# xiph/daala

Measured on AMD Instinct MI355X. Metric: 1080p all-intra transform blocks/s (filter+DCT+PVQ), higher is better.
Workload: dtype int32 (lifting DCT/filters) + f64 (PVQ search)

## Files before the change

### daala_amd/csrc/pvq_refbands.hip

```cpp
#include "../../include/daala_hip.h"
#include <math.h>
#include <stdio.h>
#include <stdlib.h>
#include <string.h>
#include "od_ctx.cuh"
#include "od_pvq_math.cuh"
#include "od_occupancy.cuh"
#include "od_krange.cuh"
#include "od_band_stage.cuh"
#include "gen/od_scan_tables.h"
#define OD_RSQ_TABLE_N 512
#define OD_RSQ_HUGE
#include "pvq_search.cuh"
#include "pvq_row.cuh"
#include "pvq_regs.cuh"

namespace {

constexpr int kMaxJobs = 8;
constexpr int kMaxItems = kMaxJobs*ODHIP_MAX_BANDS;
constexpr int kSlots = ODHIP_PVQ_REF_SLOTS;
constexpr int kUncCap = 1 << 16;
constexpr double kDefaultMargin = 1e-9;

struct RJob {
  const od_coeff *coef;
  const od_coeff *ref;
  const int16_t *qm;
  const int16_t *qm_inv;
  odhip_pvq_refband *rec;
  void *items;
  int16_t *y;
  int16_t *r16;
  int16_t *x16;
  int16_t *xr;
  const double *rate;
  int32_t *choice;
  od_coeff *dq;
  unsigned short *keys;
  unsigned *ids;
  unsigned *krange;
  long nblocks;
  int nplanes;
  int w;
  int h;
  int bs;
  int nb_bands;
  int len;
  int bw;
  int bh;
  int is_keyframe;
  int pli;
  int q[ODHIP_MAX_BANDS];
  int beta[ODHIP_MAX_BANDS];
  int off[ODHIP_MAX_BANDS + 1];
  long split_blk;
  int q2[ODHIP_MAX_BANDS];
  const int *qp;
  unsigned plane_blocks;
  const int16_t *ly;
  const int32_t *lchoice;
  const int16_t *lqmi;
  long lnblocks;
  long lsplit;
  int llen;
  int lnb;
};

__device__ __forceinline__ int job_q(const RJob &jb, int band, long blk) {
  const int q = blk >= jb.split_blk ? jb.q2[band] : jb.q[band];
  return q ? q : jb.qp[(unsigned)blk/jb.plane_blocks*ODHIP_MAX_BANDS + band];
}

__device__ __forceinline__ void lref_piece(const RJob &jb, int band, long blk, int c0, int (&rv)[8]) {
  const long lblk = blk >= jb.lsplit ? blk - jb.lsplit : blk;
  const int4 ch = reinterpret_cast<const int4 *>(jb.lchoice)[lblk*jb.lnb + band];
  uint4 y4 = make_uint4(0, 0, 0, 0);
  if (ch.y != 0) y4 = *reinterpret_cast<const uint4 *>(jb.ly + ((long)ch.x*jb.lnblocks + lblk)*jb.llen + c0);
  const uint4 q4 = *reinterpret_cast<const uint4 *>(jb.lqmi + c0);
  const unsigned yw[4] = {y4.x, y4.y, y4.z, y4.w};
  const unsigned qw[4] = {q4.x, q4.y, q4.z, q4.w};
#pragma unroll
  for (int e = 0; e < 8; e++) {
    const int yv = (int16_t)(yw[e >> 1] >> (16*(e & 1)));
    const int qmi = (int16_t)(qw[e >> 1] >> (16*(e & 1)));
    rv[e] = odq_shr_round(odq_mult16_32_q16(yv, ch.z)*qmi, ch.w);
  }
}

struct Unc;
struct PUncR {
  int job;
  int band;
  unsigned blk;
  int reserved;
  double rate[ODHIP_PVQ_REF_SLOTS + 1];
};
constexpr int kPUncCap = 1 << 14;

struct RItems : ItemTable<kMaxItems> {
  int perturb;
  double lambda;
  double margin;
  const RJob *jobs;
  unsigned *unc_count;
  Unc *unc;
  unsigned *pcount;
  struct PUncR *plist;
  double tol_scale;
  int fuse;
  int sort_weights;
#ifdef ODHIP_EXPERIMENTS
  int abl;
#endif
};

struct Unc {
  int job;
  int band;
  unsigned blk;
  int theta;
  double corr;
};

__constant__ unsigned char kRScanXY[OD_SCAN_LEN][2];

__device__ __forceinline__ long block_base(const RJob &j, long blk) {
  const int N = 4 << j.bs;
  const long per = (long)j.bw*j.bh;
  const int p = (int)(blk/per);
  const int rem = (int)(blk - p*per);
  const int by = rem/j.bw;
  const int bx = rem - by*j.bw;
  return (long)p*j.w*j.h + (long)by*N*j.w + bx*N;
}

__device__ __forceinline__ long coef_pos(const RJob &j, int c) {
  return (long)kRScanXY[c][1]*j.w + kRScanXY[c][0];
}

constexpr double kPi = 3.14159265358979323846;
constexpr double kThetaScale = 32768*2./kPi;

__device__ __forceinline__ double theta_arg(double corr) {
  return .5 + kThetaScale*acos(corr);
}

__global__ __launch_bounds__(kWave) void k_theta_probe(const double *corr, double *t, long n) {
  const long i = (long)blockIdx.x*kWave + threadIdx.x;
  if (i < n) t[i] = theta_arg(corr[i]);
}

__device__ __attribute__((aligned(16))) unsigned short gRScanPk[OD_SCAN_LEN];

struct PrepScalars {
  int32_t g, gr, cg, cgr, gain_offset;
  int icgr;
  double corr, dist0;
  bool ran;
};

__device__ __forceinline__ PrepScalars prep_scalars(int accx, int accr, double corr_sum, int xshift,
 int rshift, int q0, int beta, int cfl_enabled, int is_keyframe, int r_null) {
  PrepScalars o;
  o.cg = odq_gain_from_acc(accx, q0, beta, xshift, &o.g);
  o.cgr = odq_gain_from_acc(accr, q0, beta, rshift, &o.gr);
  if (cfl_enabled) o.cgr = 256;
  o.icgr = odq_shr_round(o.cgr, ODQ_CGAIN_SHIFT);
  o.gain_offset = o.cgr - odq_shl32(o.icgr, ODQ_CGAIN_SHIFT);
  double corr = __ddiv_rn(corr_sum,
// ... 11 lines not shown
  o.dist0 = dist0;
  o.ran = !r_null && corr > 0;
  return o;
}

__device__ __forceinline__ void householder_consts(int32_t l2r, int32_t proj, int16_t *proj_1,
 int *outshift) {
  const int l2r_shift = (odq_ilog(l2r) - 1) - 14;
  const int16_t l2r_norm = (int16_t)odq_vshr_round(l2r, l2r_shift);
  const int16_t rcp = odq_rcp(l2r_norm);
  const int proj_shift = (odq_ilog(abs(proj)) - 1) - 14;
  const int16_t proj_norm = (int16_t)odq_vshr_round(proj, proj_shift);
  *proj_1 = (int16_t)odq_mult16_16_q15(proj_norm, rcp);
  int os = 14 - proj_shift - 1 + l2r_shift;
  *outshift = os > 30 ? 30 : os;
}


constexpr int kSortBins = 256;
constexpr int kSortChunk = 2048;

__device__ __forceinline__ int od_work_bin(int pulses) {
  if (pulses < 96) return pulses;
  const int b = 96 + ((pulses - 96) >> 3);
  return b < kSortBins ? b : kSortBins - 1;
}

template <class Sink>
__device__ __forceinline__ void refb_enumerate(const RJob &jb, int band, int32_t cg, int32_t gain_offset,
 int32_t theta, int flags, double corr, Sink &sink) {
  const int n = jb.off[band + 1] - jb.off[band];
  const int beta = jb.beta[band];
  if (flags & ODHIP_REFBAND_THETA) {
    int nth = 0;
    const int gain_bound = (cg - gain_offset) >> ODQ_CGAIN_SHIFT;
    const double scale_1 = __ddiv_rn(1., kThetaScale);
    for (int i = gain_bound - 1 > 1 ? gain_bound - 1 : 1; i <= gain_bound + 1; i++) {
      const int32_t qcg = odq_shl32(i, ODQ_CGAIN_SHIFT) + gain_offset;
      const int ts = odq_pvq_compute_max_theta(qcg, beta);
      const double t = __ddiv_rn(((theta*scale_1)*2), kPi)*ts;
      int lower = (int)floor(.5 + t) - 2;
      if (lower < 0) lower = 0;
      int upper = (int)ceil(t);
      if (upper > ts - 1) upper = ts - 1;
      const int gi = i - (gain_bound - 1);
      sink.gain(gi, i, ts, lower);
      for (int j = lower; j <= upper && nth < ODHIP_PVQ_REF_SLOTS - 2; j++) {
        sink.theta(gi, i, j, ts, odq_compute_k_ref(j, n));
        nth++;
      }
    }
  }
  if ((jb.is_keyframe && jb.pli == 0) || corr < .5 || cg < odq_shl32(2, ODQ_CGAIN_SHIFT)) {
    const int gain_bound = cg >> ODQ_CGAIN_SHIFT;
    int c = 0;
    for (int i = gain_bound > 1 ? gain_bound : 1; i <= gain_bound + 1; i++) {
      sink.noref(c++, i, odq_compute_k_noref(odq_shl32(i, ODQ_CGAIN_SHIFT), n, beta));
    }
  }
}

struct KeySink {
  int kt = 0;
  int kn = 0;
  int c = 0;
  unsigned long long mt = 0;
  unsigned long long mn = 0;
  __device__ __forceinline__ void gain(int, int, int, int) {}
  __device__ __forceinline__ void theta(int, int, int, int, int k) {
    kt = k > kt ? k : kt;
    c++;
    if (k) mt |= 1ull << (k & 63);
  }
  __device__ __forceinline__ void noref(int, int, int k) {
    kn = k > kn ? k : kn;
    c++;
    if (k) mn |= 1ull << (k & 63);
  }
  __device__ __forceinline__ int work(int w) const {
    return ((w & 255)*(kt + kn) + (w >> 8 & 255)*c + (w >> 16 & 255)*(__popcll(mt) + __popcll(mn))) >> 2;
  }
};

__device__ __forceinline__ void prep_write(const RItems &it, odhip_pvq_refband *rec, int job, int band,
 long blk, int xshift, int rshift, const PrepScalars &p, int r_null, int flip, int m, int s) {
  int flags = (r_null ? ODHIP_REFBAND_R_NULL : 0) | (flip ? ODHIP_REFBAND_FLIP : 0);
  int32_t theta = 0;
  if (p.ran) {
    flags |= ODHIP_REFBAND_THETA;
    const double u = theta_arg(p.corr);
    theta = (int32_t)floor(u);
    if (fabs(u - rint(u)) < it.margin) {
      flags |= ODHIP_REFBAND_UNCERTAIN;
      if (it.perturb & 1) theta += 1;
      const unsigned slot = atomicAdd(it.unc_count, 1u);
      if (slot < (unsigned)kUncCap) {
        Unc e;
        e.job = job;
        e.band = band;
        e.blk = (unsigned)blk;
        e.theta = theta;
        e.corr = p.corr;
        it.unc[slot] = e;
      }
    }
  }
  odhip_pvq_refband o;
  o.xshift = xshift;
  o.rshift = rshift;
  o.g = p.g;
  o.gr = p.gr;
  o.cg = p.cg;
  o.cgr = p.cgr;
  o.icgr = p.icgr;
  o.gain_offset = p.gain_offset;
  o.m = (int16_t)m;
  o.s = (int8_t)s;
  o.flags = (uint8_t)flags;
  o.theta = theta;
  o.nitems = 0;
  o.ntheta = 0;
  o.corr = p.corr;
  o.dist0 = p.dist0;
  *rec = o;
  if (it.fuse == 2) {
    const RJob &jb = it.jobs[job];
    KeySink ks;
    refb_enumerate(jb, band, o.cg, o.gain_offset, o.theta, flags, o.corr, ks);
    jb.keys[(long)band*jb.nblocks + blk] = (unsigned short)(kSortBins - 1 - od_work_bin(ks.work(it.sort_weights)));
    if (ks.kt > ODHIP_PVQ_MAX_K || ks.kn > ODHIP_PVQ_MAX_K) atomicAdd(jb.krange, 1u);
  }
}

__device__ __forceinline__ uint32_t pack16(int lo, int hi) {
  return (uint32_t)(lo & 0xffff) | (uint32_t)hi << 16;
}

template <int N>
__global__ __launch_bounds__(kWave) void k_refb_prep_lane(RItems it) {
  const int item = find_item(it, blockIdx.x);
  const int job = it.job[item];
  const RJob &jb = it.jobs[job];
  const int band = it.band[item];
  const long blk = (long)(blockIdx.x - it.wg_start[item])*kWave + threadIdx.x;
  if (blk >= jb.nblocks) return;
  const int off = jb.off[band];
  const int w = jb.w;
  const int len = jb.len;
  const int nb_bands = jb.nb_bands;
  const int q0 = job_q(jb, band, blk);
  const int beta = jb.beta[band];
  const int is_keyframe = jb.is_keyframe;
  const int cfl_enabled = is_keyframe && jb.pli != 0;
  const long base = block_base(jb, blk);
  const od_coeff *x0 = jb.coef + base;
  const bool lref = jb.ly != nullptr;
  const od_coeff *r0 = lref ? jb.coef + base : jb.ref + base;
  const int16_t *qmp = jb.qm + off;
  odhip_pvq_refband *rec = jb.rec + blk*nb_bands;
  int16_t *x16o = jb.x16 + blk*len;
  int16_t *r16o = jb.r16 + blk*len;
  int16_t *xro = jb.xr + blk*len;
  int xv[N];
  int rv[N];
  int qm[N];
  if constexpr (N == 15) {
    int4 xr4[4];
    int4 rr4[4];
#pragma unroll
    for (int y = 0; y < 4; y++) {
      xr4[y] = *reinterpret_cast<const int4 *>(x0 + (long)y*w);
      rr4[y] = lref ? make_int4(0, 0, 0, 0) : *reinterpret_cast<const int4 *>(r0 + (long)y*w);
    }
#pragma unroll
    for (int i = 0; i < N; i++) {
      const int sx = OD_SCAN_XY[1 + i][0];
      const int sy = OD_SCAN_XY[1 + i][1];
      const int4 a = xr4[sy];
      const int4 b = rr4[sy];
      xv[i] = sx == 0 ? a.x : sx == 1 ? a.y : sx == 2 ? a.z : a.w;
      rv[i] = sx == 0 ? b.x : sx == 1 ? b.y : sx == 2 ? b.z : b.w;
      qm[i] = qmp[i];
    }
  }
  else if (off == 16) {
    int4 xr4[2];
    int4 rr4[2];
#pragma unroll
    for (int y = 0; y < 2; y++) {
      xr4[y] = *reinterpret_cast<const int4 *>(x0 + (long)y*w + 4);
      rr4[y] = lref ? make_int4(0, 0, 0, 0) : *reinterpret_cast<const int4 *>(r0 + (long)y*w + 4);
    }
#pragma unroll
    for (int i = 0; i < N; i++) {
      const int sx = OD_SCAN_XY[16 + (i < 8 ? i : 0)][0] - 4;
      const int sy = OD_SCAN_XY[16 + (i < 8 ? i : 0)][1];
      const int4 a = xr4[sy & 1];
      const int4 b = rr4[sy & 1];
      xv[i] = sx == 0 ? a.x : sx == 1 ? a.y : sx == 2 ? a.z : a.w;
      rv[i] = sx == 0 ? b.x : sx == 1 ? b.y : sx == 2 ? b.z : b.w;
      qm[i] = qmp[i];
    }
  }
  else if (off == 24) {
    int2 xr2[4];
    int2 rr2[4];
#pragma unroll
    for (int y = 0; y < 4; y++) {
      xr2[y] = *reinterpret_cast<const int2 *>(x0 + (long)(4 + y)*w);
      rr2[y] = lref ? make_int2(0, 0) : *reinterpret_cast<const int2 *>(r0 + (long)(4 + y)*w);
    }
#pragma unroll
    for (int i = 0; i < N; i++) {
      const int sx = OD_SCAN_XY[24 + (i < 8 ? i : 0)][0];
      const int sy = OD_SCAN_XY[24 + (i < 8 ? i : 0)][1] - 4;
      const int2 a = xr2[sy & 3];
      const int2 b = rr2[sy & 3];
      xv[i] = sx == 0 ? a.x : a.y;
      rv[i] = sx == 0 ? b.x : b.y;
      qm[i] = qmp[i];
    }
  }
  else {
#pragma unroll
    for (int i = 0; i < N; i++) {
      const long p = (long)kRScanXY[off + i][1]*w + kRScanXY[off + i][0];
      xv[i] = x0[p];
      rv[i] = lref ? 0 : r0[p];
      qm[i] = qmp[i];
    }
  }
#ifdef ODHIP_EXPERIMENTS
  const bool lref_read = lref && !(it.abl & 2);
#else
  const bool lref_read = lref;
#endif
  if (lref_read) {
    if constexpr (N == 15) {
      int lo[8];
      int hi[8];
      lref_piece(jb, band, blk, 0, lo);
      lref_piece(jb, band, blk, 8, hi);
#pragma unroll
      for (int i = 0; i < N; i++) rv[i] = i + 1 < 8 ? lo[(i + 1) & 7] : hi[(i + 1) & 7];
    }
    else {
      int pc[8];
      lref_piece(jb, band, blk, off, pc);
#pragma unroll
      for (int i = 0; i < N; i++) rv[i] = pc[i & 7];
    }
  }
  int flip = 0;
  if (cfl_enabled) {
    if (N == 15 && band == 0) {
      uint32_t xy = 0;
#pragma unroll
      for (int i = 0; i < N; i++) {
        const int32_t rq = (int32_t)((uint32_t)rv[i]*(uint32_t)qm[i]);
        const int32_t inq = (int32_t)((uint32_t)xv[i]*(uint32_t)qm[i]);
        xy += (uint32_t)((rq*(int64_t)inq) >> 30);
      }
      flip = (int32_t)xy < 0;
    }
    else flip = (rec[0].flags & ODHIP_REFBAND_FLIP) != 0;
  }
  int sx = 0;
  int sr = 0;
  int r_null = 1;
#pragma unroll
  for (int i = 0; i < N; i++) {
    if (flip) rv[i] = -rv[i];
    const int tx = (int16_t)(xv[i] >> 8);
    const int tr = (int16_t)(rv[i] >> 8);
    sx += tx*tx;
    sr += tr*tr;
    if (rv[i]) r_null = 0;
  }
  int xshift = 8 + 1 + odq_ilog(N + sx)/2 - 15;
  xshift = xshift > 0 ? xshift : 0;
  int rshift = 8 + 1 + odq_ilog(N + sr)/2 - 14;
  rshift = rshift > 0 ? rshift : 0;
  int x16[N];
  int r16[N];
  double corr = 0;
  int accx = 0;
  int accr = 0;
#pragma unroll
  for (int i = 0; i < N; i++) {
    x16[i] = (int16_t)odq_shr_round((int32_t)((uint32_t)xv[i]*(uint32_t)qm[i]), ODQ_QM_SHIFT + xshift);
    r16[i] = (int16_t)odq_shr_round((int32_t)((uint32_t)rv[i]*(uint32_t)qm[i]), ODQ_QM_SHIFT + rshift);
    corr += odq_mult16_16(x16[i], r16[i]);
    accx += x16[i]*x16[i];
    accr += r16[i]*r16[i];
  }
  const PrepScalars p = prep_scalars(accx, accr, corr, xshift, rshift, q0, beta, cfl_enabled,
   is_keyframe, r_null);
  int m = 0;
  int s = 1;
  int xr[N];
#pragma unroll
  for (int i = 0; i < N; i++) xr[i] = 0;
  if (p.ran) {
    int maxr = 0;
#pragma unroll
    for (int i = 0; i < N; i++) {
      const int a = abs(r16[i]);
      if (a > maxr) {
        maxr = a;
        m = i;
      }
    }
    int rm = 0;
#pragma unroll
    for (int i = 0; i < N; i++) if (i == m) rm = r16[i];
    s = rm > 0 ? 1 : -1;
    const int upd = (int16_t)(rm + odq_shr_round(p.gr*s, rshift));
    int32_t l2r = 0;
    int32_t proj = 0;
#pragma unroll
    for (int i = 0; i < N; i++) {
      if (i == m) r16[i] = upd;
      l2r += odq_mult16_16(r16[i], r16[i]);
      proj += odq_mult16_16(r16[i], x16[i]);
    }
    int16_t proj_1;
    int outshift;
    householder_consts(l2r, proj, &proj_1, &outshift);
    int v[N];
#pragma unroll
    for (int i = 0; i < N; i++) {
      int32_t tmp = odq_mult16_16(r16[i], proj_1);
      tmp = outshift >= 0 ? odq_shr_round(tmp, outshift) : odq_shl32(tmp, -outshift);
      v[i] = (int16_t)(x16[i] - tmp);
    }
#pragma unroll
    for (int i = 0; i < N - 1; i++) xr[i] = i < m ? v[i] : v[i + 1];
  }
#ifdef ODHIP_EXPERIMENTS
  const bool abl_nostore = (it.abl & 1) != 0;
  const bool abl_norec = (it.abl & 4) != 0;
#else
  constexpr bool abl_nostore = false;
  constexpr bool abl_norec = false;
#endif
  if (abl_nostore) {
  }
  else if (N == 15) {
    uint4 *xo = reinterpret_cast<uint4 *>(x16o);
    uint4 *ro = reinterpret_cast<uint4 *>(r16o);
    uint4 *xro4 = reinterpret_cast<uint4 *>(xro);
    xo[0] = make_uint4(pack16(0, x16[0]), pack16(x16[1], x16[2]), pack16(x16[3], x16[4]),
     pack16(x16[5], x16[6]));
    xo[1] = make_uint4(pack16(x16[7], x16[8]), pack16(x16[9], x16[10]), pack16(x16[11], x16[12]),
     pack16(x16[13], x16[N - 1]));
    ro[0] = make_uint4(pack16(0, r16[0]), pack16(r16[1], r16[2]), pack16(r16[3], r16[4]),
     pack16(r16[5], r16[6]));
    ro[1] = make_uint4(pack16(r16[7], r16[8]), pack16(r16[9], r16[10]), pack16(r16[11], r16[12]),
     pack16(r16[13], r16[N - 1]));
    xro4[0] = make_uint4(pack16(0, xr[0]), pack16(xr[1], xr[2]), pack16(xr[3], xr[4]),
     pack16(xr[5], xr[6]));
    xro4[1] = make_uint4(pack16(xr[7], xr[8]), pack16(xr[9], xr[10]), pack16(xr[11], xr[12]),
     pack16(xr[13], 0));
  }
  else {
    *reinterpret_cast<uint4 *>(x16o + off) = make_uint4(pack16(x16[0], x16[1]), pack16(x16[2], x16[3]),
     pack16(x16[4], x16[5]), pack16(x16[6], x16[7]));
    *reinterpret_cast<uint4 *>(r16o + off) = make_uint4(pack16(r16[0], r16[1]), pack16(r16[2], r16[3]),
     pack16(r16[4], r16[5]), pack16(r16[6], r16[7]));
    *reinterpret_cast<uint4 *>(xro + off) = make_uint4(pack16(xr[0], xr[1]), pack16(xr[2], xr[3]),
     pack16(xr[4], xr[5]), pack16(xr[6], 0));
  }
  if (!abl_norec) prep_write(it, rec + band, job, band, blk, xshift, rshift, p, r_null, flip, m, s);
}

template <int E, int G>
__global__ __launch_bounds__(kWave) void k_refb_prep_row(RItems it) {
  constexpr int n = G*E;
  __shared__ unsigned short s_scan[n];
  const int item = find_item(it, blockIdx.x);
  const int job = it.job[item];
  const RJob &jb = it.jobs[job];
  const int band = it.band[item];
  const int off = jb.off[band];
  const int lane = threadIdx.x;
  for (int j = lane; j < n; j += kWave) s_scan[j] = gRScanPk[off + j];
  __syncthreads();
  const int row = lane/G;
  const int l = lane%G;
  const long nblocks = jb.nblocks;
  const long blk0 = (long)(blockIdx.x - it.wg_start[item])*(kWave/G) + row;
  const bool live = blk0 < nblocks;
  const long blk = live ? blk0 : nblocks - 1;
  const int w = jb.w;
  const int len = jb.len;
  const int nb_bands = jb.nb_bands;
  const int q0 = job_q(jb, band, blk);
  const int beta = jb.beta[band];
  const int is_keyframe = jb.is_keyframe;
  const int cfl_enabled = is_keyframe && jb.pli != 0;
  const long base = block_base(jb, blk);
  const od_coeff *x0 = jb.coef + base;
  const bool lref = jb.ly != nullptr;
  const od_coeff *r0 = lref ? jb.coef + base : jb.ref + base;
  const int16_t *qmp = jb.qm + off + l*E;
  odhip_pvq_refband *rec = jb.rec + blk*nb_bands;
  int16_t *x16o = jb.x16 + blk*len + off;
  int16_t *r16o = jb.r16 + blk*len + off;
  int16_t *xro = jb.xr + blk*len + off;
  const int flip = cfl_enabled ? (rec[0].flags & ODHIP_REFBAND_FLIP) != 0 : 0;
  int xv[E];
  int rv[E];
  int qm[E];
  int sx = 0;
  int sr = 0;
  int nz = 0;
#pragma unroll
  for (int e = 0; e < E; e++) {
    const int pk = s_scan[l*E + e];
    const long p = (long)(pk >> 8)*w + (pk & 255);
    xv[e] = x0[p];
    const int r = lref ? 0 : r0[p];
    rv[e] = flip ? -r : r;
    qm[e] = qmp[e];
  }
  if (lref) {
    static_assert(E == 8, "one 16-byte piece of the luma stage's pulses per lane");
    int pc[8];
    lref_piece(jb, band, blk, off + l*E, pc);
#pragma unroll
    for (int e = 0; e < E; e++) rv[e] = flip ? -pc[e] : pc[e];
  }
#pragma unroll
  for (int e = 0; e < E; e++) {
    const int tx = (int16_t)(xv[e] >> 8);
    const int tr = (int16_t)(rv[e] >> 8);
    sx += tx*tx;
    sr += tr*tr;
    nz |= rv[e] != 0;
  }
  sx = grp_sum<G>(sx);
  sr = grp_sum<G>(sr);
  const int r_null = grp_max<G>(nz) == 0;
  int xshift = 8 + 1 + odq_ilog(n + sx)/2 - 15;
  xshift = xshift > 0 ? xshift : 0;
  int rshift = 8 + 1 + odq_ilog(n + sr)/2 - 14;
  rshift = rshift > 0 ? rshift : 0;
  int x16[E];
  int r16[E];
  double corr = 0;
  int accx = 0;
  int accr = 0;
#pragma unroll
  for (int e = 0; e < E; e++) {
    x16[e] = (int16_t)odq_shr_round((int32_t)((uint32_t)xv[e]*(uint32_t)qm[e]), ODQ_QM_SHIFT + xshift);
    r16[e] = (int16_t)odq_shr_round((int32_t)((uint32_t)rv[e]*(uint32_t)qm[e]), ODQ_QM_SHIFT + rshift);
    corr += odq_mult16_16(x16[e], r16[e]);
    accx += x16[e]*x16[e];
    accr += r16[e]*r16[e];
  }
  corr = grp_sum<G>(corr);
  accx = grp_sum<G>(accx);
  accr = grp_sum<G>(accr);
  const PrepScalars p = prep_scalars(accx, accr, corr, xshift, rshift, q0, beta, cfl_enabled,
   is_keyframe, r_null);
  int m = 0;
  int s = 1;
  if (p.ran) {
    int ba = -1;
    int bi = 0;
#pragma unroll
    for (int e = 0; e < E; e++) {
      const int a = abs(r16[e]);
      if (a > ba) {
        ba = a;
        bi = l*E + e;
      }
    }
#define OD_ARGMAX_STEP(CTRL) \
    { \
      const int oa = row_mov<CTRL>(ba); \
      const int oi = row_mov<CTRL>(bi); \
      const bool take = oa > ba || (oa == ba && oi < bi); \
      ba = take ? oa : ba; \
      bi = take ? oi : bi; \
    }
    OD_ARGMAX_STEP(OD_DPP_XOR1)
    OD_ARGMAX_STEP(OD_DPP_XOR2)
    if (G == 16) {
      OD_ARGMAX_STEP(OD_DPP_HALF_MIRROR)
      OD_ARGMAX_STEP(OD_DPP_MIRROR)
    }
#undef OD_ARGMAX_STEP
    m = bi;
    int rm = 0;
#pragma unroll
    for (int e = 0; e < E; e++) if (l*E + e == m) rm = r16[e];
    rm = grp_sum<G>(rm);
    s = rm > 0 ? 1 : -1;
    const int upd = (int16_t)(rm + odq_shr_round(p.gr*s, rshift));
    int32_t l2r = 0;
    int32_t proj = 0;
#pragma unroll
    for (int e = 0; e < E; e++) {
      if (l*E + e == m) r16[e] = upd;
      l2r += odq_mult16_16(r16[e], r16[e]);
      proj += odq_mult16_16(r16[e], x16[e]);
    }
    l2r = grp_sum<G>(l2r);
    proj = grp_sum<G>(proj);
    int16_t proj_1;
    int outshift;
    householder_consts(l2r, proj, &proj_1, &outshift);
#pragma unroll
    for (int e = 0; e < E; e++) {
      const int i = l*E + e;
      int32_t tmp = odq_mult16_16(r16[e], proj_1);
      tmp = outshift >= 0 ? odq_shr_round(tmp, outshift) : odq_shl32(tmp, -outshift);
      const int16_t v = (int16_t)(x16[e] - tmp);
      if (live && i != m) xro[i - (i > m)] = v;
    }
  }
  if (live) {
    if constexpr (E == 8) {
      *reinterpret_cast<uint4 *>(x16o + l*E) = make_uint4(pack16(x16[0], x16[1]),
       pack16(x16[2], x16[3]), pack16(x16[4], x16[5]), pack16(x16[6], x16[7]));
      *reinterpret_cast<uint4 *>(r16o + l*E) = make_uint4(pack16(r16[0], r16[1]),
       pack16(r16[2], r16[3]), pack16(r16[4], r16[5]), pack16(r16[6], r16[7]));
    }
    else {
#pragma unroll
      for (int e = 0; e < E; e += 2) {
        *reinterpret_cast<uint32_t *>(x16o + l*E + e) = pack16(x16[e], x16[e + 1]);
        *reinterpret_cast<uint32_t *>(r16o + l*E + e) = pack16(r16[e], r16[e + 1]);
      }
    }
    if (l == 0) prep_write(it, rec + band, job, band, blk, xshift, rshift, p, r_null, flip, m, s);
  }
}


struct ItemPtr {
  int4 *head;
  int4 *tail;
  int4 *res;
  long stride;
};

__device__ __forceinline__ ItemPtr item_ptr(const RJob &jb, int band, long blk) {
  ItemPtr p;
  const long plane = (long)jb.nb_bands*kSlots*jb.nblocks;
  p.head = reinterpret_cast<int4 *>(jb.items) + (long)band*kSlots*jb.nblocks + blk;
  p.tail = p.head + plane;
  p.res = p.tail + plane;
  p.stride = jb.nblocks;
  return p;
}

__device__ __forceinline__ void refb_candidates(const RJob &jb, int band, long blk,
 int theta_override, int4 (*stage)[kWave]) {
  const int lane = threadIdx.x;
  odhip_pvq_refband *rp = jb.rec + blk*jb.nb_bands + band;
  odhip_pvq_refband r = *rp;
  if (theta_override >= 0) r.theta = theta_override;
  const int n = jb.off[band + 1] - jb.off[band];
  const int beta = jb.beta[band];
  const ItemPtr ip = item_ptr(jb, band, blk);
  int nitems = 0;
  int kmax_theta = 0;
  int kmax_noref = 0;
  if (r.flags & ODHIP_REFBAND_THETA) {
    const int gain_bound = (r.cg - r.gain_offset) >> ODQ_CGAIN_SHIFT;
    const double scale_1 = __ddiv_rn(1., kThetaScale);
    for (int i = gain_bound - 1 > 1 ? gain_bound - 1 : 1; i <= gain_bound + 1; i++) {
      const int32_t qcg = odq_shl32(i, ODQ_CGAIN_SHIFT) + r.gain_offset;
      const int ts = odq_pvq_compute_max_theta(qcg, beta);
      const double t = __ddiv_rn(((r.theta*scale_1)*2), kPi)*ts;
      int lower = (int)floor(.5 + t) - 2;
      if (lower < 0) lower = 0;
      int upper = (int)ceil(t);
      if (upper > ts - 1) upper = ts - 1;
      for (int j = lower; j <= upper && nitems < kSlots - 2; j++) {
        const int4 c = make_int4(i, j, ts, odq_compute_k_ref(j, n));
        kmax_theta = c.w > kmax_theta ? c.w : kmax_theta;
        int pos = nitems;
        while (pos > 0) {
          const int4 q = stage[pos - 1][lane];
          const int cmp = q.w == c.w ? q.x - c.x : q.w - c.w;
          if (cmp <= 0) break;
          stage[pos][lane] = q;
          pos--;
        }
        stage[pos][lane] = c;
        nitems++;
      }
    }
  }
  const int ntheta = nitems;
  int flags = r.flags & ~ODHIP_REFBAND_NOREF;
  if ((jb.is_keyframe && jb.pli == 0) || r.corr < .5 || r.cg < odq_shl32(2, ODQ_CGAIN_SHIFT)) {
    flags |= ODHIP_REFBAND_NOREF;
    const int gain_bound = r.cg >> ODQ_CGAIN_SHIFT;
    for (int i = gain_bound > 1 ? gain_bound : 1; i <= gain_bound + 1; i++) {
      const int kk = odq_compute_k_noref(odq_shl32(i, ODQ_CGAIN_SHIFT), n, beta);
      stage[nitems][lane] = make_int4(i, -1, 0, kk);
      kmax_noref = kk > kmax_noref ? kk : kmax_noref;
      nitems++;
    }
  }
  for (int i = 0; i < nitems; i++) ip.head[i*ip.stride] = stage[i][lane];
  int4 v;
  v.x = (int)((uint32_t)(uint16_t)r.m | (uint32_t)(uint8_t)r.s << 16 | (uint32_t)flags << 24);
  v.y = r.theta;
  v.z = nitems;
  v.w = ntheta;
  reinterpret_cast<int4 *>(rp)[2] = v;
  jb.keys[(long)band*jb.nblocks + blk] = (unsigned short)(kSortBins - 1 - od_work_bin(kmax_theta + kmax_noref));
}

__global__ __launch_bounds__(kWave) void k_refb_cands(RItems it) {
// ... 1558 lines not shown
int ref_state(RefState **out) {
  ODHIP_CTX_OR_RETURN(ctx);
  RefState *st = odhip_ctx_state<RefState>(ctx, ODHIP_SLOT_REFBANDS);
  if (!st->tabs.d.p) {
    int rc = st->tabs.alloc();
    if (!rc) rc = st->counters.alloc();
    if (!rc) rc = st->unc.alloc(kUncCap);
    if (!rc) rc = st->sort.alloc();
    if (!rc) rc = st->plist.alloc(kPUncCap);
    if (rc) return rc;
  }
  st->streams.serial = ctx->serial != 0;
  st->margin = ctx->theta_margin > 0 ? ctx->theta_margin : kDefaultMargin;
  st->perturb = ctx->theta_perturb != 0;
  st->tol_scale = ctx->price_tol_scale > 0 ? ctx->price_tol_scale : 1.;
  *out = st;
  return ODHIP_SUCCESS;
}
#define REF_STATE_OR_RETURN(st) STAGE_STATE_OR_RETURN(RefState, ref_state, st)

int stage_jobs(RefState &st, const odhip_pvq_refjob *jobs, int njobs, JobMode mode, RJob *host,
 hipStream_t s) {
  if (!jobs || njobs <= 0 || njobs > kMaxJobs) return ODHIP_EINVAL;
  int rc = upload_tables();
  if (rc) return rc;
  for (int i = 0; i < njobs; i++) {
    rc = fill_job(host[i], jobs[i], mode);
    if (rc) return rc;
    host[i].krange = st.counters.d.p + 2;
  }
  if (mode == kJobBands) {
    rc = st.sort.place(host, njobs, s);
    if (rc) return rc;
  }
  return st.tabs.upload(host, njobs, s);
}

int sort_weights(void) {
  static const int w = [] {
    int p = 4, c = 4, s = 8;
    const char *e = ODHIP_EXP_ENV("ODHIP_SORT_W");
    if (e) sscanf(e, "%d,%d,%d", &p, &c, &s);
    return (p & 255) | (c & 255) << 8 | (s & 255) << 16;
  }();
  return w;
}

void items_begin(RItems &it, const RefState &st, double lambda) {
  memset(&it, 0, sizeof(it));
  it.lambda = lambda;
  it.margin = st.margin;
  it.perturb = st.perturb;
  it.jobs = st.tabs.cur;
  it.unc_count = st.unc_count();
  it.unc = st.unc.p;
  it.pcount = st.pcount();
  it.plist = st.plist.p;
  it.tol_scale = st.tol_scale;
  it.sort_weights = sort_weights();
#ifdef ODHIP_EXPERIMENTS
  static const int abl = [] {
    const char *e = getenv("ODHIP_REFB_ABL");
    return e ? atoi(e) : 0;
  }();
  it.abl = abl;
#endif
}

enum RefStage {
  kStageRecords = 0,
  kStageLanePriced = 1,
  kStageDecided = 2
};

void launch_prep(const RefState &st, const RJob *host, int njobs, double lambda, RefStage stage, hipStream_t s) {
  RItems pi;
  const auto prep = [&](void (*kernel)(RItems), int size, long per_wg) {
    items_begin(pi, st, lambda);
    pi.fuse = stage;
    if (size) items_add_size(pi, host, njobs, size, per_wg, 1);
    else for (int j = 0; j < njobs; j++) items_add(pi, j, 0, (host[j].nblocks + per_wg - 1)/per_wg);
    if (pi.nitems) kernel<<<pi.wg_start[pi.nitems], kWave, 0, s>>>(pi);
  };
  prep(k_refb_prep_lane<15>, 0, kWave);
  prep(k_refb_prep_lane<8>, 8, kWave);
  prep(k_refb_prep_row<8, 4>, 32, 16);
  prep(k_refb_prep_row<8, 16>, 128, 4);
}

int sort_blocks(RefState &st, const RJob *host, int njobs, hipStream_t s) {
  return st.sort.run(host, st.tabs.cur, njobs, s);
}

struct RefSearch {
  int size;
  int on;
  int per_wg;
  bool row;
};
constexpr RefSearch kRefSearches[4] = {{128, 0, 4, true}, {32, 1, 16, true}, {15, 2, kWave, false},
 {8, 2, kWave, false}};

void launch_search(RefState &st, RItems &it, const RefSearch &r, RefStage stage, hipStream_t s) {
  if (stage == kStageDecided) items_heavy_first(it);
  const int wgs = it.wg_start[it.nitems];
  const int groups = (wgs + kSearchWaves - 1)/kSearchWaves;
  const auto regs = [&](auto priced) {
    for_band_size(r.size, [&](auto size) {
      constexpr int N = decltype(size)::value;
      if constexpr (N <= 15) k_refb_search_regs<N, decltype(priced)::value><<<wgs, kWave, 0, s>>>(it);
    });
  };
  const auto launch = [&] {
    if (r.row) {
      for_band_size(r.size, [&](auto size) {
        constexpr int N = decltype(size)::value;
        if constexpr (N >= 32) {
          if (stage == kStageDecided) k_refb_lean_row<8, N/8><<<groups, kSearchThreads, 0, s>>>(it);
          else k_refb_search_row<8, N/8><<<wgs, kWave, 0, s>>>(it);
        }
      });
    }
    else if (stage == kStageDecided) {
      for_band_size(r.size, [&](auto size) {
        constexpr int N = decltype(size)::value;
        if constexpr (N <= 15) k_refb_lean_lane<N><<<groups, kSearchThreads, 0, s>>>(it);
      });
    }
    else if (stage == kStageLanePriced) regs(std::true_type());
    else regs(std::false_type());
  };
  if (r.size == 128) st.prof.around(s, launch);
  else launch();
}

int launch_searches(RefState &st, const RJob *host, int njobs, double lambda, RefStage stage, hipStream_t s) {
  const bool lane_only = stage != kStageDecided && ODHIP_EXP_ENV("ODHIP_PVQ_REF_LANE") != nullptr;
  hipStream_t side[2] = {s, s};
  if (st.streams.fork(s, side) != ODHIP_SUCCESS) return ODHIP_EFAULT;
  const hipStream_t streams[3] = {s, side[0], side[1]};
  RItems it;
  for (const RefSearch &r : kRefSearches) {
    items_begin(it, st, lambda);
    if (r.row && !lane_only && odhip_env_force_seq()) it.perturb |= 2;
    items_add_size(it, host, njobs, r.size, lane_only ? kWave : r.per_wg);
    if (it.nitems && !lane_only) launch_search(st, it, r, stage, streams[r.on]);
#ifdef ODHIP_EXPERIMENTS
    if (it.nitems && lane_only) {
      k_refb_search<<<it.wg_start[it.nitems], kWave, (size_t)2*r.size*kWave*sizeof(unsigned short), streams[r.on]>>>(it);
    }
#endif
  }
  if (st.streams.join(s, side) != ODHIP_SUCCESS) return ODHIP_EFAULT;
  return ODHIP_SUCCESS;
}

int ref_bands(const odhip_pvq_refjob *jobs, int njobs, double pvq_norm_lambda, odhip_stream stream, RefStage stage) {
  hipStream_t s = (hipStream_t)stream;
  REF_STATE_OR_RETURN(st);
  RJob host[kMaxJobs];
  int rc = stage_jobs(st, jobs, njobs, kJobBands, host, s);
  if (rc) return rc;
  ODHIP_TRY(hipMemsetAsync(st.unc_count(), 0, (stage != kStageRecords ? 2 : 1)*sizeof(unsigned), s));
  st.lean = stage == kStageDecided;
  RItems it;
  items_begin(it, st, pvq_norm_lambda);
  items_add_size(it, host, njobs, 0, kWave);
  if (!it.nitems) return ODHIP_SUCCESS;
// ... 294 lines not shown
```

Measured before the change: 1.162 billion.

## Fuse band-0 and 8-coefficient band prep into one corner kernel per block

Replaces the two separate lane prep launches (band 0 with 15 coefficients, and the two 8-coefficient bands) with a single k_refb_prep_corner kernel that loads the 8x8 top-left corner once per block and prepares all three bands. The CfL flip sign is computed in registers and passed to the 8-coefficient bands instead of being read back from the band-0 record, which also removes the ordering dependency between the launches. It uses explicit global and constant address-space loads, and loads the lref choice and pulse data branch-free with a mask. The fused kernel carries more live registers per thread, which may lower occupancy, and it depends on a fixed band layout enforced by a static_assert.

New measurement: 1.178 billion (median of 6 runs). +1.4%, better.

```diff
diff --git a/daala_amd/csrc/pvq_refbands.hip b/daala_amd/csrc/pvq_refbands.hip
--- a/daala_amd/csrc/pvq_refbands.hip
+++ b/daala_amd/csrc/pvq_refbands.hip
@@ -72,12 +72,11 @@
   return q ? q : jb.qp[(unsigned)blk/jb.plane_blocks*ODHIP_MAX_BANDS + band];
 }
 
-__device__ __forceinline__ void lref_piece(const RJob &jb, int band, long blk, int c0, int (&rv)[8]) {
-  const long lblk = blk >= jb.lsplit ? blk - jb.lsplit : blk;
-  const int4 ch = reinterpret_cast<const int4 *>(jb.lchoice)[lblk*jb.lnb + band];
-  uint4 y4 = make_uint4(0, 0, 0, 0);
-  if (ch.y != 0) y4 = *reinterpret_cast<const uint4 *>(jb.ly + ((long)ch.x*jb.lnblocks + lblk)*jb.llen + c0);
-  const uint4 q4 = *reinterpret_cast<const uint4 *>(jb.lqmi + c0);
+__device__ __forceinline__ long lref_block(const RJob &jb, long blk) {
+  return blk >= jb.lsplit ? blk - jb.lsplit : blk;
+}
+
+__device__ __forceinline__ void lref_dequant(const int4 &ch, const uint4 &y4, const uint4 &q4, int (&rv)[8]) {
   const unsigned yw[4] = {y4.x, y4.y, y4.z, y4.w};
   const unsigned qw[4] = {q4.x, q4.y, q4.z, q4.w};
 #pragma unroll
@@ -86,6 +85,14 @@
     const int qmi = (int16_t)(qw[e >> 1] >> (16*(e & 1)));
     rv[e] = odq_shr_round(odq_mult16_32_q16(yv, ch.z)*qmi, ch.w);
   }
+}
+
+__device__ __forceinline__ void lref_piece(const RJob &jb, int band, long blk, int c0, int (&rv)[8]) {
+  const long lblk = lref_block(jb, blk);
+  const int4 ch = reinterpret_cast<const int4 *>(jb.lchoice)[lblk*jb.lnb + band];
+  uint4 y4 = make_uint4(0, 0, 0, 0);
+  if (ch.y != 0) y4 = *reinterpret_cast<const uint4 *>(jb.ly + ((long)ch.x*jb.lnblocks + lblk)*jb.llen + c0);
+  lref_dequant(ch, y4, *reinterpret_cast<const uint4 *>(jb.lqmi + c0), rv);
 }
 
 struct Unc;
@@ -263,7 +270,7 @@
   }
 };
 
-__device__ __forceinline__ void prep_write(const RItems &it, odhip_pvq_refband *rec, int job, int band,
+__device__ __forceinline__ void prep_write(const RItems &it, const RJob &jb, odhip_pvq_refband *rec, int job, int band,
  long blk, int xshift, int rshift, const PrepScalars &p, int r_null, int flip, int m, int s) {
   int flags = (r_null ? ODHIP_REFBAND_R_NULL : 0) | (flip ? ODHIP_REFBAND_FLIP : 0);
   int32_t theta = 0;
@@ -305,7 +312,6 @@
   o.dist0 = p.dist0;
   *rec = o;
   if (it.fuse == 2) {
-    const RJob &jb = it.jobs[job];
     KeySink ks;
     refb_enumerate(jb, band, o.cg, o.gain_offset, o.theta, flags, o.corr, ks);
     jb.keys[(long)band*jb.nblocks + blk] = (unsigned short)(kSortBins - 1 - od_work_bin(ks.work(it.sort_weights)));
@@ -317,135 +323,127 @@
   return (uint32_t)(lo & 0xffff) | (uint32_t)hi << 16;
 }
 
+constexpr bool lane_band_layout_ok() {
+  for (int bs = 0; bs < 5; bs++) {
+    const int nb = OD_NBANDS[bs];
+    if (OD_BAND_OFFS[bs][0] != 1 || OD_BAND_OFFS[bs][1] != 16 || (nb > 1 && nb < 3)) return false;
+    for (int b = 1; b < nb; b++) {
+      const bool lane = OD_BAND_OFFS[bs][b + 1] - OD_BAND_OFFS[bs][b] == 8;
+      if (lane != (OD_BAND_OFFS[bs][b] == 8 + 8*b && b <= 2)) return false;
+    }
+  }
+  return true;
+}
+static_assert(lane_band_layout_ok(), "k_refb_prep_corner: band 0 at 1..15, 8-coefficient bands at 16 and 24 only");
+
+struct CornerSegs {
+  int4 b0[4];
+  int4 b1[2];
+  int2 b2[4];
+};
+
+typedef int od_int4v __attribute__((ext_vector_type(4)));
+typedef int od_int2v __attribute__((ext_vector_type(2)));
+
+__device__ __forceinline__ int4 global_load4(const void *p) {
+  const od_int4v v = *(const __attribute__((address_space(1))) od_int4v *)p;
+  return make_int4(v.x, v.y, v.z, v.w);
+}
+
+__device__ __forceinline__ int2 global_load2(const void *p) {
+  const od_int2v v = *(const __attribute__((address_space(1))) od_int2v *)p;
+  return make_int2(v.x, v.y);
+}
+
+typedef const __attribute__((address_space(4))) int16_t *od_const_i16;
+
+__device__ __forceinline__ od_const_i16 const_table(const int16_t *p) {
+  return (od_const_i16)p;
+}
+
+__device__ __forceinline__ uint4 const_load4(const int16_t *p) {
+  const od_int4v v = *(const __attribute__((address_space(4))) od_int4v *)p;
+  return make_uint4((unsigned)v.x, (unsigned)v.y, (unsigned)v.z, (unsigned)v.w);
+}
+
+__device__ __forceinline__ void corner_load(const od_coeff *p, int w, bool more, CornerSegs &s) {
+#pragma unroll
+  for (int y = 0; y < 4; y++) s.b0[y] = global_load4(p + (long)y*w);
+#pragma unroll
+  for (int y = 0; y < 2; y++) s.b1[y] = more ? global_load4(p + (long)y*w + 4) : make_int4(0, 0, 0, 0);
+#pragma unroll
+  for (int y = 0; y < 4; y++) s.b2[y] = more ? global_load2(p + (long)(4 + y)*w) : make_int2(0, 0);
+}
+
+__device__ __forceinline__ int4 lref_choice(const RJob &jb, int band, long lblk) {
+  return global_load4(jb.lchoice + (lblk*jb.lnb + band)*4);
+}
+
+__device__ __forceinline__ uint4 lref_pulses(const RJob &jb, const int4 &ch, long lblk, int c0) {
+  const long slot = ch.y != 0 ? ch.x : 0;
+  const int4 y4 = global_load4(jb.ly + (slot*jb.lnblocks + lblk)*jb.llen + c0);
+  const unsigned keep = ch.y != 0 ? ~0u : 0u;
+  return make_uint4(y4.x & keep, y4.y & keep, y4.z & keep, y4.w & keep);
+}
+
+__device__ __forceinline__ void corner_zero(CornerSegs &s) {
+#pragma unroll
+  for (int y = 0; y < 4; y++) {
+    s.b0[y] = make_int4(0, 0, 0, 0);
+    s.b1[y & 1] = make_int4(0, 0, 0, 0);
+    s.b2[y] = make_int2(0, 0);
+  }
+}
+
+__device__ __forceinline__ int int4_at(const int4 &a, int i) {
+  return i == 0 ? a.x : i == 1 ? a.y : i == 2 ? a.z : a.w;
+}
+
+__device__ __forceinline__ void unpack_band0(const int4 (&s)[4], int (&v)[15]) {
+#pragma unroll
+  for (int i = 0; i < 15; i++) v[i] = int4_at(s[OD_SCAN_XY[1 + i][1]], OD_SCAN_XY[1 + i][0]);
+}
+
+__device__ __forceinline__ void unpack_band1(const int4 (&s)[2], int (&v)[8]) {
+#pragma unroll
+  for (int i = 0; i < 8; i++) v[i] = int4_at(s[OD_SCAN_XY[16 + i][1] & 1], OD_SCAN_XY[16 + i][0] - 4);
+}
+
+__device__ __forceinline__ void unpack_band2(const int2 (&s)[4], int (&v)[8]) {
+#pragma unroll
+  for (int i = 0; i < 8; i++) {
+    const int2 a = s[(OD_SCAN_XY[24 + i][1] - 4) & 3];
+    v[i] = OD_SCAN_XY[24 + i][0] == 0 ? a.x : a.y;
+  }
+}
+
+__device__ __forceinline__ int cfl_flip15(const int (&xv)[15], const int (&rv)[15], od_const_i16 qmp) {
+  uint32_t xy = 0;
+#pragma unroll
+  for (int i = 0; i < 15; i++) {
+    const int qm = qmp[i];
+    const int32_t rq = (int32_t)((uint32_t)rv[i]*(uint32_t)qm);
+    const int32_t inq = (int32_t)((uint32_t)xv[i]*(uint32_t)qm);
+    xy += (uint32_t)((rq*(int64_t)inq) >> 30);
+  }
+  return (int32_t)xy < 0;
+}
+
 template <int N>
-__global__ __launch_bounds__(kWave) void k_refb_prep_lane(RItems it) {
-  const int item = find_item(it, blockIdx.x);
-  const int job = it.job[item];
-  const RJob &jb = it.jobs[job];
-  const int band = it.band[item];
-  const long blk = (long)(blockIdx.x - it.wg_start[item])*kWave + threadIdx.x;
-  if (blk >= jb.nblocks) return;
-  const int off = jb.off[band];
-  const int w = jb.w;
+__device__ __forceinline__ void prep_lane_band(const RItems &it, const RJob &jb, int job, int band, long blk,
+ int off, const int (&xv)[N], int (&rv)[N], int flip) {
   const int len = jb.len;
-  const int nb_bands = jb.nb_bands;
   const int q0 = job_q(jb, band, blk);
   const int beta = jb.beta[band];
   const int is_keyframe = jb.is_keyframe;
   const int cfl_enabled = is_keyframe && jb.pli != 0;
-  const long base = block_base(jb, blk);
-  const od_coeff *x0 = jb.coef + base;
-  const bool lref = jb.ly != nullptr;
-  const od_coeff *r0 = lref ? jb.coef + base : jb.ref + base;
-  const int16_t *qmp = jb.qm + off;
-  odhip_pvq_refband *rec = jb.rec + blk*nb_bands;
+  const od_const_i16 qmp = const_table(jb.qm + off);
   int16_t *x16o = jb.x16 + blk*len;
   int16_t *r16o = jb.r16 + blk*len;
   int16_t *xro = jb.xr + blk*len;
-  int xv[N];
-  int rv[N];
   int qm[N];
-  if constexpr (N == 15) {
-    int4 xr4[4];
-    int4 rr4[4];
-#pragma unroll
-    for (int y = 0; y < 4; y++) {
-      xr4[y] = *reinterpret_cast<const int4 *>(x0 + (long)y*w);
-      rr4[y] = lref ? make_int4(0, 0, 0, 0) : *reinterpret_cast<const int4 *>(r0 + (long)y*w);
-    }
-#pragma unroll
-    for (int i = 0; i < N; i++) {
-      const int sx = OD_SCAN_XY[1 + i][0];
-      const int sy = OD_SCAN_XY[1 + i][1];
-      const int4 a = xr4[sy];
-      const int4 b = rr4[sy];
-      xv[i] = sx == 0 ? a.x : sx == 1 ? a.y : sx == 2 ? a.z : a.w;
-      rv[i] = sx == 0 ? b.x : sx == 1 ? b.y : sx == 2 ? b.z : b.w;
-      qm[i] = qmp[i];
-    }
-  }
-  else if (off == 16) {
-    int4 xr4[2];
-    int4 rr4[2];
-#pragma unroll
-    for (int y = 0; y < 2; y++) {
-      xr4[y] = *reinterpret_cast<const int4 *>(x0 + (long)y*w + 4);
-      rr4[y] = lref ? make_int4(0, 0, 0, 0) : *reinterpret_cast<const int4 *>(r0 + (long)y*w + 4);
-    }
-#pragma unroll
-    for (int i = 0; i < N; i++) {
-      const int sx = OD_SCAN_XY[16 + (i < 8 ? i : 0)][0] - 4;
-      const int sy = OD_SCAN_XY[16 + (i < 8 ? i : 0)][1];
-      const int4 a = xr4[sy & 1];
-      const int4 b = rr4[sy & 1];
-      xv[i] = sx == 0 ? a.x : sx == 1 ? a.y : sx == 2 ? a.z : a.w;
-      rv[i] = sx == 0 ? b.x : sx == 1 ? b.y : sx == 2 ? b.z : b.w;
-      qm[i] = qmp[i];
-    }
-  }
-  else if (off == 24) {
-    int2 xr2[4];
-    int2 rr2[4];
-#pragma unroll
-    for (int y = 0; y < 4; y++) {
-      xr2[y] = *reinterpret_cast<const int2 *>(x0 + (long)(4 + y)*w);
-      rr2[y] = lref ? make_int2(0, 0) : *reinterpret_cast<const int2 *>(r0 + (long)(4 + y)*w);
-    }
-#pragma unroll
-    for (int i = 0; i < N; i++) {
-      const int sx = OD_SCAN_XY[24 + (i < 8 ? i : 0)][0];
-      const int sy = OD_SCAN_XY[24 + (i < 8 ? i : 0)][1] - 4;
-      const int2 a = xr2[sy & 3];
-      const int2 b = rr2[sy & 3];
-      xv[i] = sx == 0 ? a.x : a.y;
-      rv[i] = sx == 0 ? b.x : b.y;
-      qm[i] = qmp[i];
-    }
-  }
-  else {
-#pragma unroll
-    for (int i = 0; i < N; i++) {
-      const long p = (long)kRScanXY[off + i][1]*w + kRScanXY[off + i][0];
-      xv[i] = x0[p];
-      rv[i] = lref ? 0 : r0[p];
-      qm[i] = qmp[i];
-    }
-  }
-#ifdef ODHIP_EXPERIMENTS
-  const bool lref_read = lref && !(it.abl & 2);
-#else
-  const bool lref_read = lref;
-#endif
-  if (lref_read) {
-    if constexpr (N == 15) {
-      int lo[8];
-      int hi[8];
-      lref_piece(jb, band, blk, 0, lo);
-      lref_piece(jb, band, blk, 8, hi);
-#pragma unroll
-      for (int i = 0; i < N; i++) rv[i] = i + 1 < 8 ? lo[(i + 1) & 7] : hi[(i + 1) & 7];
-    }
-    else {
-      int pc[8];
-      lref_piece(jb, band, blk, off, pc);
-#pragma unroll
-      for (int i = 0; i < N; i++) rv[i] = pc[i & 7];
-    }
-  }
-  int flip = 0;
-  if (cfl_enabled) {
-    if (N == 15 && band == 0) {
-      uint32_t xy = 0;
-#pragma unroll
-      for (int i = 0; i < N; i++) {
-        const int32_t rq = (int32_t)((uint32_t)rv[i]*(uint32_t)qm[i]);
-        const int32_t inq = (int32_t)((uint32_t)xv[i]*(uint32_t)qm[i]);
-        xy += (uint32_t)((rq*(int64_t)inq) >> 30);
-      }
-      flip = (int32_t)xy < 0;
-    }
-    else flip = (rec[0].flags & ODHIP_REFBAND_FLIP) != 0;
-  }
+#pragma unroll
+  for (int i = 0; i < N; i++) qm[i] = qmp[i];
   int sx = 0;
   int sr = 0;
   int r_null = 1;
@@ -552,8 +550,168 @@
     *reinterpret_cast<uint4 *>(xro + off) = make_uint4(pack16(xr[0], xr[1]), pack16(xr[2], xr[3]),
      pack16(xr[4], xr[5]), pack16(xr[6], 0));
   }
-  if (!abl_norec) prep_write(it, rec + band, job, band, blk, xshift, rshift, p, r_null, flip, m, s);
-}
+  if (!abl_norec) {
+    prep_write(it, jb, jb.rec + blk*jb.nb_bands + band, job, band, blk, xshift, rshift, p, r_null, flip, m, s);
+  }
+}
+
+__global__ __launch_bounds__(kWave) void k_refb_prep_corner(RItems it) {
+  const int item = find_item(it, blockIdx.x);
+  const int job = __builtin_amdgcn_readfirstlane(it.job[item]);
+  const RJob jb = it.jobs[job];
+  const long blk = (long)(blockIdx.x - it.wg_start[item])*kWave + threadIdx.x;
+  if (blk >= jb.nblocks) return;
+  const bool more = jb.nb_bands > 1;
+  const int w = jb.w;
+  const long base = block_base(jb, blk);
+  const bool lref = jb.ly != nullptr;
+#ifdef ODHIP_EXPERIMENTS
+  const bool lref_read = lref && !(it.abl & 2);
+#else
+  const bool lref_read = lref;
+#endif
+  const long lblk = lref_block(jb, blk);
+  int4 ch[3];
+  uint4 ly[4];
+#pragma unroll
+  for (int b = 0; b < 3; b++) ch[b] = make_int4(0, 0, 0, 0);
+#pragma unroll
+  for (int i = 0; i < 4; i++) ly[i] = make_uint4(0, 0, 0, 0);
+  if (lref_read) {
+    ch[0] = lref_choice(jb, 0, lblk);
+    if (more) {
+      ch[1] = lref_choice(jb, 1, lblk);
+      ch[2] = lref_choice(jb, 2, lblk);
+    }
+  }
+  CornerSegs xs;
+  CornerSegs rs;
+  corner_load(jb.coef + base, w, more, xs);
+  if (!lref) corner_load(jb.ref + base, w, more, rs);
+  else {
+    corner_zero(rs);
+    if (lref_read) {
+      ly[0] = lref_pulses(jb, ch[0], lblk, 0);
+      ly[1] = lref_pulses(jb, ch[0], lblk, 8);
+      if (more) {
+        ly[2] = lref_pulses(jb, ch[1], lblk, 16);
+        ly[3] = lref_pulses(jb, ch[2], lblk, 24);
+      }
+    }
+  }
+  int xv[15];
+  int rv[15];
+  unpack_band0(xs.b0, xv);
+  unpack_band0(rs.b0, rv);
+  if (lref_read) {
+    int lo[8];
+    int hi[8];
+    lref_dequant(ch[0], ly[0], const_load4(jb.lqmi), lo);
+    lref_dequant(ch[0], ly[1], const_load4(jb.lqmi + 8), hi);
+#pragma unroll
+    for (int i = 0; i < 15; i++) rv[i] = i + 1 < 8 ? lo[(i + 1) & 7] : hi[(i + 1) & 7];
+  }
+  const int cfl_enabled = jb.is_keyframe && jb.pli != 0;
+  const int flip = cfl_enabled ? cfl_flip15(xv, rv, const_table(jb.qm + jb.off[0])) : 0;
+  if (more) {
+    int xb[8];
+    int rb[8];
+    unpack_band1(xs.b1, xb);
+    unpack_band1(rs.b1, rb);
+    if (lref_read) lref_dequant(ch[1], ly[2], const_load4(jb.lqmi + 16), rb);
+    prep_lane_band<8>(it, jb, job, 1, blk, 16, xb, rb, flip);
+    unpack_band2(xs.b2, xb);
+    unpack_band2(rs.b2, rb);
+    if (lref_read) lref_dequant(ch[2], ly[3], const_load4(jb.lqmi + 24), rb);
+    prep_lane_band<8>(it, jb, job, 2, blk, 24, xb, rb, flip);
+  }
+  prep_lane_band<15>(it, jb, job, 0, blk, jb.off[0], xv, rv, flip);
+}
+
+#ifdef ODHIP_EXPERIMENTS
+template <int N>
+__global__ __launch_bounds__(kWave) void k_refb_prep_lane(RItems it) {
+  const int item = find_item(it, blockIdx.x);
+  const int job = it.job[item];
+  const RJob &jb = it.jobs[job];
+  const int band = it.band[item];
+  const long blk = (long)(blockIdx.x - it.wg_start[item])*kWave + threadIdx.x;
+  if (blk >= jb.nblocks) return;
+  const int off = jb.off[band];
+  const int w = jb.w;
+  const long base = block_base(jb, blk);
+  const od_coeff *x0 = jb.coef + base;
+  const bool lref = jb.ly != nullptr;
+  const od_coeff *r0 = lref ? jb.coef + base : jb.ref + base;
+  int xv[N];
+  int rv[N];
+  if constexpr (N == 15) {
+    int4 xs[4];
+    int4 rs[4];
+#pragma unroll
+    for (int y = 0; y < 4; y++) {
+      xs[y] = *reinterpret_cast<const int4 *>(x0 + (long)y*w);
+      rs[y] = lref ? make_int4(0, 0, 0, 0) : *reinterpret_cast<const int4 *>(r0 + (long)y*w);
+    }
+    unpack_band0(xs, xv);
+    unpack_band0(rs, rv);
+  }
+  else {
+    if (off == 16) {
+      int4 xs[2];
+      int4 rs[2];
+#pragma unroll
+      for (int y = 0; y < 2; y++) {
+        xs[y] = *reinterpret_cast<const int4 *>(x0 + (long)y*w + 4);
+        rs[y] = lref ? make_int4(0, 0, 0, 0) : *reinterpret_cast<const int4 *>(r0 + (long)y*w + 4);
+      }
+      unpack_band1(xs, xv);
+      unpack_band1(rs, rv);
+    }
+    else if (off == 24) {
+      int2 xs[4];
+      int2 rs[4];
+#pragma unroll
+      for (int y = 0; y < 4; y++) {
+        xs[y] = *reinterpret_cast<const int2 *>(x0 + (long)(4 + y)*w);
+        rs[y] = lref ? make_int2(0, 0) : *reinterpret_cast<const int2 *>(r0 + (long)(4 + y)*w);
+      }
+      unpack_band2(xs, xv);
+      unpack_band2(rs, rv);
+    }
+    else {
+#pragma unroll
+      for (int i = 0; i < N; i++) {
+        const long p = (long)kRScanXY[off + i][1]*w + kRScanXY[off + i][0];
+        xv[i] = x0[p];
+        rv[i] = lref ? 0 : r0[p];
+      }
+    }
+  }
+  if (lref && !(it.abl & 2)) {
+    if constexpr (N == 15) {
+      int lo[8];
+      int hi[8];
+      lref_piece(jb, band, blk, 0, lo);
+      lref_piece(jb, band, blk, 8, hi);
+#pragma unroll
+      for (int i = 0; i < N; i++) rv[i] = i + 1 < 8 ? lo[(i + 1) & 7] : hi[(i + 1) & 7];
+    }
+    else {
+      int pc[8];
+      lref_piece(jb, band, blk, off, pc);
+#pragma unroll
+      for (int i = 0; i < N; i++) rv[i] = pc[i & 7];
+    }
+  }
+  int flip = 0;
+  if (jb.is_keyframe && jb.pli != 0) {
+    if constexpr (N == 15) flip = cfl_flip15(xv, rv, const_table(jb.qm + off));
+    else flip = (jb.rec[blk*jb.nb_bands].flags & ODHIP_REFBAND_FLIP) != 0;
+  }
+  prep_lane_band<N>(it, jb, job, band, blk, off, xv, rv, flip);
+}
+#endif
 
 template <int E, int G>
 __global__ __launch_bounds__(kWave) void k_refb_prep_row(RItems it) {
@@ -716,7 +874,7 @@
         *reinterpret_cast<uint32_t *>(r16o + l*E + e) = pack16(r16[e], r16[e + 1]);
       }
     }
-    if (l == 0) prep_write(it, rec + band, job, band, blk, xshift, rshift, p, r_null, flip, m, s);
+    if (l == 0) prep_write(it, jb, rec + band, job, band, blk, xshift, rshift, p, r_null, flip, m, s);
   }
 }
 
@@ -2441,8 +2599,15 @@
     else for (int j = 0; j < njobs; j++) items_add(pi, j, 0, (host[j].nblocks + per_wg - 1)/per_wg);
     if (pi.nitems) kernel<<<pi.wg_start[pi.nitems], kWave, 0, s>>>(pi);
   };
-  prep(k_refb_prep_lane<15>, 0, kWave);
-  prep(k_refb_prep_lane<8>, 8, kWave);
+#ifdef ODHIP_EXPERIMENTS
+  static const bool split = getenv("ODHIP_REFB_PREP_SPLIT") != nullptr;
+  if (split) {
+    prep(k_refb_prep_lane<15>, 0, kWave);
+    prep(k_refb_prep_lane<8>, 8, kWave);
+  }
+  else
+#endif
+  prep(k_refb_prep_corner, 0, kWave);
   prep(k_refb_prep_row<8, 4>, 32, 16);
   prep(k_refb_prep_row<8, 16>, 128, 4);
 }
```
